# honglu2875/hironaka

Measured on AMD Instinct MI355X. Metric: env-steps/sec at dim=3, max_pts=20, batch=65536; 1/2/4/8 GPUs, higher is better.
Workload: dtype f32

## Files before the change

### hironaka_amd/csrc/hk_duo_kernel.h

```cpp
#pragma once

#include "hk_fast_kernel.h"

namespace hk {

constexpr int kDuoGames = kWave / 2;

__device__ __forceinline__ int duo_other_i(int v) { return qperm_i<0xB1>(v); }
__device__ __forceinline__ float duo_other(float v) { return __int_as_float(duo_other_i(__float_as_int(v))); }

template <int M, int D>
struct DuoGeom {
  using G = FastGeom<M, D>;
  static constexpr int CH = (G::C + 1) / 2;
  static constexpr int QH = (kDuoGames * G::Q + kWave - 1) / kWave;
  static constexpr bool kLean = CH * D <= 30;
};

template <int M, int D>
struct DuoSlabRegs {
  typename VecOf<FastGeom<M, D>::W>::type v[DuoGeom<M, D>::QH];
};

template <int M, int D, bool CONTIG>
__device__ __forceinline__ void duo_slab_issue_impl(DuoSlabRegs<M, D>& r, const float* base, int64_t in_stride,
                                                    int ngames, int lane) {
  using G = FastGeom<M, D>;
  using V = typename VecOf<G::W>::type;
  const int total = ngames * G::Q;
#pragma unroll
  for (int it = 0; it < DuoGeom<M, D>::QH; ++it) {
    int q = lane + it * kWave;
    q = q < total ? q : total - 1;
    r.v[it] = *reinterpret_cast<const V*>(base + slab_chunk_global<M, D, CONTIG>(q, in_stride));
  }
}

template <int M, int D>
__device__ __forceinline__ void duo_slab_issue(DuoSlabRegs<M, D>& r, const float* in, int64_t in_stride, int64_t g0,
                                               int ngames, int lane) {
  const float* base = in + g0 * in_stride;
  if (in_stride == FastGeom<M, D>::N) duo_slab_issue_impl<M, D, true>(r, base, in_stride, ngames, lane);
  else duo_slab_issue_impl<M, D, false>(r, base, in_stride, ngames, lane);
}

template <int M, int D>
__device__ __forceinline__ void duo_slab_commit(DuoSlabRegs<M, D>& r, float* lds, int ngames, int lane) {
  using G = FastGeom<M, D>;
  using V = typename VecOf<G::W>::type;
  const int total = ngames * G::Q;
#pragma unroll
  for (int it = 0; it < DuoGeom<M, D>::QH; ++it) asm volatile("" : "+v"(r.v[it]));
#pragma unroll
  for (int it = 0; it < DuoGeom<M, D>::QH; ++it) {
    const int q = lane + it * kWave;
    if (q < total) *reinterpret_cast<V*>(lds + slab_chunk_lds<M, D>(q)) = r.v[it];
  }
}

constexpr int kStorePlain = 0, kStoreNT = 1, kStoreWT = 2;

template <int M, int D, bool CONTIG, int kBatch, int ST = kStorePlain>
__device__ __forceinline__ void duo_store_slab_impl(const float* lds, float* base, int64_t out_stride, int ngames,
                                                    int lane) {
  using G = FastGeom<M, D>;
  using V = typename VecOf<G::W>::type;
  constexpr int QH = DuoGeom<M, D>::QH;
  constexpr bool kWT = ST == kStoreWT && CONTIG && G::W == 4;
  const int total = ngames * G::Q;
#pragma unroll
  for (int i0 = 0; i0 < QH; i0 += kBatch) {
    V v[kBatch];
#pragma unroll
    for (int u = 0; u < kBatch; ++u) {
      int q = lane + (i0 + u) * kWave;
      q = q < kDuoGames * G::Q ? q : kDuoGames * G::Q - 1;
      v[u] = *reinterpret_cast<const V*>(lds + slab_chunk_lds<M, D>(q));
    }
#pragma unroll
    for (int u = 0; u < kBatch; ++u) asm volatile("" : "+v"(v[u]));
    if constexpr (kWT) {
      typedef unsigned int vu4 __attribute__((ext_vector_type(4)));
      const uint64_t b = (uint64_t)base;
      const uint32_t blo = __builtin_amdgcn_readfirstlane((uint32_t)b), bhi = __builtin_amdgcn_readfirstlane((uint32_t)(b >> 32));
      const int bytes = __builtin_amdgcn_readfirstlane(total * G::W * (int)sizeof(float));
      const auto rsrc = __builtin_amdgcn_make_buffer_rsrc((void*)(((uint64_t)bhi << 32) | blo), 0, bytes, 0x00020000);
#pragma unroll
      for (int u = 0; u < kBatch; ++u) {
        const int q = lane + (i0 + u) * kWave;
        if (i0 + u < QH && q < total)
          __builtin_amdgcn_raw_buffer_store_b128(__builtin_bit_cast(vu4, v[u]), rsrc, q * G::W * (int)sizeof(float), 0,
                                                 16);
      }
    } else {
#pragma unroll
      for (int u = 0; u < kBatch; ++u) {
        const int q = lane + (i0 + u) * kWave;
        if (i0 + u < QH && q < total) {
          V* dst = reinterpret_cast<V*>(base + slab_chunk_global<M, D, CONTIG>(q, out_stride));
          if constexpr (ST != kStorePlain) __builtin_nontemporal_store(v[u], dst);
          else *dst = v[u];
        }
      }
    }
  }
}

template <int M, int D, int kBatch = DuoGeom<M, D>::QH, int ST = kStorePlain>
__device__ inline void duo_store_slab(const float* lds, float* out, int64_t out_stride, int64_t g0, int ngames,
                                      int lane) {
  float* base = out + g0 * out_stride;
  if (out_stride == FastGeom<M, D>::N) duo_store_slab_impl<M, D, true, kBatch, ST>(lds, base, out_stride, ngames, lane);
  else duo_store_slab_impl<M, D, false, kBatch, ST>(lds, base, out_stride, ngames, lane);
}

struct DuoLadder {
  static constexpr int next_bucket(int nb) { return nb < 6 ? nb + 1 : nb + 2; }
};

template <int M, int CH, int D, int SB = CH>
__device__ __forceinline__ void duo_gather_slots(float (&q)[CH * D], const float* mine, uint32_t mask, int smax, int h) {
  mask = h ? (mask & (mask - 1)) : mask;
  unrolled_while<0, SB>([&](auto sc) {
    constexpr int s = decltype(sc)::value;
    if (s >= smax) return false;
    const bool has = mask != 0;
    const float* row = mine + (has ? mask_first(mask) : 0) * D;
    mask &= mask - 1;
    mask &= mask - 1;
#pragma unroll
    for (int k = 0; k < D; ++k) {
      const float v = row[k];
      q[s * D + k] = has ? v : INFINITY;
    }
    return true;
  });
}

template <int CH, int D, int NB, int SB = NB>
__device__ __forceinline__ void duo_gather_level(float (&q)[CH * D], const float* mine, const float* hole, uint32_t mask,
                                                 int h) {
  mask = h ? (mask & (mask - 1)) : mask;
  const float* row[NB];
#pragma unroll
  for (int s = 0; s < NB; ++s) {
    row[s] = mask != 0 ? mine + mask_first(mask) * D : hole;
    mask &= mask - 1;
    mask &= mask - 1;
  }
#pragma unroll
  for (int s = 0; s < NB; ++s)
#pragma unroll
    for (int k = 0; k < D; ++k) q[s * D + k] = row[s][k];
#pragma unroll
  for (int e = NB * D; e < SB * D; ++e) q[e] = INFINITY;
}

template <int M, int CH, int D, bool LEVELS, int SB = CH>
__device__ __forceinline__ void duo_gather(float (&q)[CH * D], const float* mine, const float* hole, uint32_t mask,
                                           int smax, int h) {
  if constexpr (LEVELS) {
    StagesFor<DuoLadder, SB>::run(smax, [&](auto nb) {
      duo_gather_level<CH, D, decltype(nb)::value, SB>(q, mine, hole, mask, h);
      return 0;
    });
  } else {
    duo_gather_slots<M, CH, D, SB>(q, mine, mask, smax, h);
  }
}

template <int CH, int D, int NB>
__device__ __forceinline__ uint32_t duo_scatter_level(const float (&q)[CH * D], float* mine, uint32_t mask, int h) {
  mask = h ? (mask & (mask - 1)) : mask;
  uint32_t alive = 0;
#pragma unroll
  for (int s = 0; s < NB; ++s) {
    if (mask != 0 && q[s * D] < INFINITY) {
      const int slot = mask_first(mask);
      alive |= 1u << slot;
      float* row = mine + slot * D;
#pragma unroll
      for (int k = 0; k < D; ++k) row[k] = q[s * D + k];
    }
    mask &= mask - 1;
    mask &= mask - 1;
  }
  return alive;
}

template <int M, int CH, int D, int SB = CH>
__device__ __forceinline__ uint32_t duo_scatter(const float (&q)[CH * D], float* mine, uint32_t mask, int smax, int h) {
  mask = h ? (mask & (mask - 1)) : mask;
  uint32_t alive = 0;
  unrolled_while<0, SB>([&](auto sc) {
    constexpr int s = decltype(sc)::value;
    if (s >= smax) return false;
    if (mask != 0 && q[s * D] < INFINITY) {
      const int slot = mask_first(mask);
      alive |= 1u << slot;
      float* row = mine + slot * D;
#pragma unroll
      for (int k = 0; k < D; ++k) row[k] = q[s * D + k];
    }
    mask &= mask - 1;
    mask &= mask - 1;
    return true;
  });
  return lanes_or<2>(alive);
}

template <int D>
__device__ __forceinline__ void duo_pad_rows(float* mine, uint32_t dead, float pad, int h) {
  dead = h ? (dead & (dead - 1)) : dead;
  while (dead != 0) {
    float* row = mine + mask_first(dead) * D;
#pragma unroll
    for (int k = 0; k < D; ++k) row[k] = pad;
    dead &= dead - 1;
    dead &= dead - 1;
  }
}

template <int M, int D>
__device__ __forceinline__ void duo_scan_half(const float* mine, float fill, int h, uint32_t& live, bool& ok) {
  static_assert(M <= 32, "the game's mask is one word");
  constexpr int C = (M + 1) / 2;
  const int i0 = h * C;
  const float* base = mine + i0 * D;
  uint32_t mask = 0;
  ok = true;
  const uint32_t fill_bits = __float_as_uint(fill);
#pragma unroll
  for (int r = 0; r < C; ++r) {
    const bool valid = (M % 2 == 0) || r + 1 < C || h == 0;
    uint32_t hi = __float_as_uint(base[r * D]), lo = hi;
#pragma unroll
    for (int k = 1; k < D; ++k) {
      const uint32_t u = __float_as_uint(base[r * D + k]);
      hi = u > hi ? u : hi;
      lo = u < lo ? u : lo;
    }
    const bool ge = hi < 0x7F800000u;
    const bool fl = (lo == fill_bits) && (hi == fill_bits);
    ok &= (ge | fl | !valid);
    mask |= (ge && valid) ? (1u << r) : 0u;
  }
  mask <<= i0;
  live = lanes_or<2>(mask);
}

template <int CH, int D, int NB>
__device__ __forceinline__ void d_newton(float (&q)[CH * D], int h) {
  float acc[NB], oth[NB];
#pragma unroll
  for (int i = 0; i + 1 < NB; ++i) {
#pragma unroll
    for (int j = i + 1; j < NB; ++j) {
      float t, u;
      diff_extrema<D>(&q[i * D], &q[j * D], t, u);
      const float vi = (t > 0.0f) ? -u : 1.0f;
      acc[j] = (i == 0) ? t : hk_fmin(acc[j], t);
      acc[i] = (i == 0 && j == 1) ? vi : hk_fmin(acc[i], vi);
    }
    __builtin_amdgcn_sched_barrier(0);
  }
  const bool late = h != 0;
#pragma unroll
  for (int b = 0; b < NB; ++b) {
    float o[D];
#pragma unroll
    for (int k = 0; k < D; ++k) o[k] = duo_other(q[b * D + k]);
    {
      float t, u;
      diff_extrema<D>(&q[b * D], o, t, u);
      const float va = (t > 0.0f || late) ? -u : 1.0f;
      acc[b] = (NB == 1) ? va : hk_fmin(acc[b], va);
      oth[b] = (u < 0.0f || !late) ? t : 1.0f;
    }
#pragma unroll
    for (int a = 0; a < b; ++a) {
      float t, u;
      diff_extrema<D>(&q[a * D], o, t, u);
      oth[b] = hk_fmin(oth[b], t);
      acc[a] = hk_fmin(acc[a], (t > 0.0f) ? -u : 1.0f);
    }
    __builtin_amdgcn_sched_barrier(0);
  }
#pragma unroll
  for (int r = 0; r < NB; ++r) {
    const bool r0 = acc[r] <= 0.0f, r1 = duo_other(oth[r]) <= 0.0f;
    const bool removed = r0 || r1;
#pragma unroll
    for (int k = 0; k < D; ++k) q[r * D + k] = removed ? INFINITY : q[r * D + k];
  }
}

template <int CH, int D, int NB, bool BIN = false>
__device__ __forceinline__ int d_stages(float (&q)[CH * D], const float (&c)[D], int axis, int np, int h,
                                        unsigned flags, unsigned stages, uint32_t cmask = 0) {
  if (stages & HK_STAGE_SHIFT) {
    if constexpr (BIN) b_shift_mask<CH, D, NB>(q, cmask, axis, np, flags);
    else b_shift<CH, D, NB>(q, c, axis, np, flags);
  }
  if (stages & HK_STAGE_REPOSITION) reposition<2, CH, D, NB, BIN>(q, flags);
  if (stages & HK_STAGE_NEWTON) d_newton<CH, D, NB>(q, h);
  if (stages & HK_STAGE_RESCALE) rescale<2, CH, D, NB>(q, flags);
  return live_rows<2, CH, D, NB>(q);
}

template <int CH, int D, int NB, bool BIN = false>
struct DuoStagesFor {
  static constexpr int kNext = DuoLadder::next_bucket(NB);
  static __device__ __forceinline__ int run(float (&q)[CH * D], int smax, const float (&c)[D], int axis, int np,
                                            int h, unsigned flags, unsigned stages, uint32_t cmask = 0) {
    if constexpr (NB >= CH) {
      return d_stages<CH, D, CH, BIN>(q, c, axis, np, h, flags, stages, cmask);
    } else {
      if (smax <= NB) return d_stages<CH, D, NB, BIN>(q, c, axis, np, h, flags, stages, cmask);
      return DuoStagesFor<CH, D, kNext, BIN>::run(q, smax, c, axis, np, h, flags, stages, cmask);
    }
  }
};

template <int CH, int D>
__device__ __forceinline__ void duo_ranks_first(const float (&q)[CH * D], int smax, int (&rank)[CH]) {
#pragma unroll
  for (int s = 0; s < CH; ++s) rank[s] = 0;
  unrolled_while<0, CH>([&](auto bc) {
    constexpr int b = decltype(bc)::value;
    if (b >= smax) return false;
    float o[D];
#pragma unroll
    for (int k = 0; k < D; ++k) o[k] = duo_other(q[b * D + k]);
    const bool live_o = o[0] < INFINITY, live_b = q[b * D] < INFINITY;
    unrolled_while<0, CH>([&](auto ac) {
      constexpr int a = decltype(ac)::value;
      if (a >= smax) return false;
      rank[a] += (live_o && key_gt<D, kKeyFirst>(o, &q[a * D])) ? 1 : 0;
      if (a != b) rank[a] += (live_b && key_gt<D, kKeyFirst>(&q[b * D], &q[a * D])) ? 1 : 0;
      return true;
    });
    return true;
  });
}

template <int CH, int D>
__device__ __forceinline__ void duo_scatter_ranked(const float (&q)[CH * D], float* mine, const int (&rank)[CH], int smax) {
  unrolled_while<0, CH>([&](auto sc) {
    constexpr int s = decltype(sc)::value;
    if (s >= smax) return false;
    if (q[s * D] < INFINITY) {
      float* row = mine + rank[s] * D;
#pragma unroll
      for (int k = 0; k < D; ++k) row[k] = q[s * D + k];
    }
    return true;
  });
}

struct DuoPolicyCache {
  U4 r;
  uint32_t pair = 0xFFFFFFFFu;
};

__device__ inline void duo_policy_words(uint64_t gg, uint32_t step, uint64_t seed, DuoPolicyCache& cache, int h,
                                        uint32_t& host_word, uint32_t& agent_word) {
  const uint32_t block = step >> 2, pair = block >> 1;
  if (cache.pair != pair) {
    cache.r = philox4x32((uint32_t)gg, (uint32_t)(gg >> 32), (pair << 1) | (uint32_t)h, kStreamPolicy, seed);
    cache.pair = pair;
  }
  const uint32_t mine = u4_word(cache.r, step & 3u);
  const bool own = (int)(block & 1u) == h;
  uint32_t theirs = (uint32_t)duo_other_i((int)mine);
  asm volatile("" : "+v"(theirs));
  const uint32_t w = own ? mine : theirs;
  host_word = w & 0xFFFF0000u;
  agent_word = w << 16;
}

constexpr int kDuoZeilDpp = 6;

template <int CH, int D, int NB>
__device__ __forceinline__ int duo_zeillinger(const float (&q)[CH * D], int h, float* mine, int smax) {
  constexpr bool KEEP = NB <= kDuoZeilDpp;
  ZeilBest<D> best;
#pragma unroll
  for (int k = 0; k < D; ++k) best.bd[k] = 0.0f;
  if constexpr (KEEP) {
    float p[NB * D];
#pragma unroll
    for (int e = 0; e < NB * D; ++e) p[e] = duo_other(q[e]);
#pragma unroll
    for (int a = 0; a < NB; ++a) {
#pragma unroll
      for (int b = a + 1; b < NB; ++b)
        zeil_pair_cmp<D, true, false>(best, &q[a * D], &q[b * D], true, (128 * a + 2 * b) + 65 * h);
#pragma unroll
      for (int b = a; b < NB; ++b)
        zeil_pair_cmp<D, true>(best, &q[a * D], &p[b * D], (b > a) | (h == 0), (128 * a + 2 * b + 1) + 63 * h);
      if constexpr (NB > 3) __builtin_amdgcn_sched_barrier(0);
    }
  } else {
    __syncthreads();
#pragma unroll
    for (int s = 0; s < NB; ++s)
#pragma unroll
      for (int k = 0; k < D; ++k) mine[(2 * s + h) * D + k] = q[s * D + k];
    __syncthreads();
    const int n = 2 * smax;
    ZeilBest<D> second;
#pragma nounroll
    for (int i = h; i + 1 < n; i += 2) {
      float pi[D];
#pragma unroll
      for (int k = 0; k < D; ++k) pi[k] = mine[i * D + k];
#pragma nounroll
      for (int j = i + 1; j < n; j += 2) {
        float pj[D], pk[D];
        const int j2 = (j + 1 < n) ? j + 1 : j;
#pragma unroll
        for (int k = 0; k < D; ++k) {
          pj[k] = mine[j * D + k];
          pk[k] = mine[j2 * D + k];
        }
        zeil_pair2<D>(best, second, pi, pj, 64 * i + j, pi, pk, 64 * i + j + 1);
      }
    }
    zeil_merge<D, false>(best, second);
  }
  {
    ZeilBest<D> o;
    o.hi = (uint32_t)duo_other_i((int)best.hi);
    o.lo = (uint32_t)duo_other_i((int)best.lo);
    if constexpr (KEEP) {
#pragma unroll
      for (int k = 0; k < D; ++k) o.bd[k] = duo_other(best.bd[k]);
    }
    zeil_merge<D, KEEP>(best, o);
  }
  const bool have = best.have();
  if constexpr (!KEEP) {
    const int i = have ? (int)((best.lo & 0xFFFFu) >> 6) : 0, j = have ? (int)(best.lo & 63u) : 0;
#pragma unroll
    for (int k = 0; k < D; ++k) best.bd[k] = mine[i * D + k] - mine[j * D + k];
    __syncthreads();
  }
  int lo = 0, hi = 0;
  float vlo = best.bd[0], vhi = best.bd[0];
#pragma unroll
  for (int k = 1; k < D; ++k) {
    if (best.bd[k] < vlo) { vlo = best.bd[k]; lo = k; }
    if (best.bd[k] > vhi) { vhi = best.bd[k]; hi = k; }
  }
  if (!have || lo == hi) return 0;
  return encode_mask((1u << lo) | (1u << hi));
}

constexpr int kDuoPreBlocks = 6;

template <int D>
__device__ __forceinline__ void duo_policy_fill(uint8_t* act, uint64_t gg, uint32_t wb0, int nb, uint64_t seed,
                                                int host_policy, int agent_policy, int gi, int h) {
  static_assert(D <= 5 && D <= kPolicyShortDim, "an action travels as a byte; four steps per Philox block");
  auto put = [&](const U4& r, int b) {
    int cls, axis;
    uint32_t mask;
#pragma unroll
    for (int k = 0; k < 4; ++k) {
      const uint32_t w = u4_word(r, k);
      policy_from_words<D>(w & 0xFFFF0000u, w << 16, host_policy, agent_policy, cls, axis, mask, 0);
      act[(4 * b + k) * kDuoGames + gi] = (uint8_t)(mask | ((uint32_t)axis << 5));
    }
  };
#pragma nounroll
  for (int i = 0; i < kDuoPreBlocks; i += 4) {
    if (i >= nb) break;
    const int b0 = i + h, b1 = b0 + 2;
    if (i + 2 < nb) {
      const U4 r0 = philox4x32((uint32_t)gg, (uint32_t)(gg >> 32), wb0 + (uint32_t)b0, kStreamPolicy, seed);
      const U4 r1 = philox4x32((uint32_t)gg, (uint32_t)(gg >> 32), wb0 + (uint32_t)b1, kStreamPolicy, seed);
      put(r0, b0);
      if (b1 < kDuoPreBlocks) put(r1, b1);
    } else {
      const U4 r0 = philox4x32((uint32_t)gg, (uint32_t)(gg >> 32), wb0 + (uint32_t)b0, kStreamPolicy, seed);
      if (b0 < kDuoPreBlocks) put(r0, b0);
    }
  }
}

template <int M, int D, int MODE, int HOT = kHotNone, bool ACTS = false, bool ZEIL = false>
__global__ __launch_bounds__(kWave, 2) void duo_kernel(const float* in0, int64_t in_stride0, int batch0,
                                                       const Params prm) {
  static_assert(!ACTS || MODE == kModeRollout, "the small records ride on the plain rollout");
  static_assert(!ZEIL || (MODE == kModeRollout && HOT == kHotNone && !ACTS), "Zeillinger's host: plain rollouts");
  constexpr bool kRec = MODE == kModeRolloutRec;
  constexpr bool kRoll = MODE == kModeRollout || kRec;
  constexpr bool kPartialPublish = MODE == kModeRollout && !ZEIL && DuoGeom<M, D>::kLean;
  constexpr bool kLevelDeal = MODE == kModeRollout && DuoGeom<M, D>::kLean;
  using G = FastGeom<M, D>;
  constexpr int CH = DuoGeom<M, D>::CH;
  static_assert(M <= 32, "the live mask of a game travels as 32 bits");
  __shared__ __align__(16) float lds[kDuoGames * G::S];
  __shared__ float cbuf[kDuoGames * D];
  __shared__ float hole_row[D];
  __shared__ __align__(16) uint8_t pol[(MODE == kModeRollout) ? (4 * kDuoPreBlocks + 1) * kDuoGames : 16];
  const int lane = threadIdx.x;
  const int h = lane & 1, gi = lane >> 1;
  const int64_t g0 = (int64_t)blockIdx.x * kDuoGames;
  const int64_t left = (int64_t)batch0 - g0;
  const int ngames = (int)(left < kDuoGames ? left : kDuoGames);
  const bool active = gi < ngames;
  const bool leader = active && h == 0;
  const int64_t g = g0 + gi;
#ifdef HK_DUO_PROBE
  __shared__ int32_t probe_buf[24];
  if (lane < 24) probe_buf[lane] = 0;
  const long long probe_t0 = wall_clock64();
  long long probe_t1 = 0, probe_t2 = 0;
  int probe_steps = 0, probe_smax = 0;
#endif
  const bool has_ids = kRoll && prm.game_ids != nullptr;
  uint32_t raw_id = 0;
  if (has_ids && active) raw_id = (uint32_t)prm.game_ids[g];
  __builtin_amdgcn_sched_barrier(0);
  DuoSlabRegs<M, D> slab;
  duo_slab_issue<M, D>(slab, in0, in_stride0, g0, ngames, lane);
  __builtin_amdgcn_sched_barrier(0);
  const uint64_t gg = prm.game_offset + (has_ids ? (uint64_t)raw_id : (uint64_t)g);
  uint32_t pol_b0 = prm.step_offset >> 2;
  const uint32_t pol_last = (prm.steps > 0) ? (prm.step_offset + (uint32_t)prm.steps - 1u) >> 2 : pol_b0;
  if constexpr (MODE == kModeRollout && !ZEIL) {
    const uint32_t nb = pol_last - pol_b0 + 1u;
    duo_policy_fill<D>(pol, gg, pol_b0, (int)(nb < (uint32_t)kDuoPreBlocks ? nb : (uint32_t)kDuoPreBlocks), prm.seed,
                       HOT ? (int)HK_HOST_RANDOM : prm.host_policy,
                       (HOT == kHotJax) ? (int)HK_AGENT_RANDOM
                                        : (HOT == kHotTorch) ? (int)HK_AGENT_RANDOM_LEGAL : prm.agent_policy, gi, h);
  }
#ifdef HK_DUO_PROBE
  if (lane == 0) probe_buf[21] = (int32_t)wall_clock64();
#endif
  float* mine = lds + gi * G::S;
  const float pad = (float)prm.pad;
  const unsigned flags = (HOT == kHotJax) ? (unsigned)HK_SEM_JAX : (HOT == kHotTorch) ? kHotTorchFlags : prm.flags;
  const unsigned stages = HOT ? (unsigned)(HK_STAGE_SHIFT | HK_STAGE_REPOSITION | HK_STAGE_NEWTON) : prm.stages;
  const float fill = ((flags & HK_SEM_MASK) == HK_SEM_JAX) ? -1.0f : pad;
  const int nsteps = kRoll ? prm.steps : 1;
  constexpr bool kEndSort = MODE == kModeRollout && HOT == kHotNone;
  const bool end_sort = kEndSort && nsteps > 0 && (stages & HK_STAGE_NEWTON) &&
                        ((flags & HK_SEM_MASK) == HK_SEM_LIST || (flags & HK_FLAG_COMPACT_SORTED));
  bool rescale_pending = false;
  PolicyCache pcache;
  DuoPolicyCache dcache;
  float c[D];
  int axis_in = -1;
#pragma unroll
  for (int k = 0; k < D; ++k) c[k] = 0.0f;
  RawActions<D> raw;
  const bool fetch_actions = !kRoll && (stages & HK_STAGE_SHIFT) && active;
  if (fetch_actions) fast_fetch_actions<D>(prm, g, M, raw);
  duo_slab_commit<M, D>(slab, lds, ngames, lane);
  if (kLevelDeal && lane < D) hole_row[lane] = INFINITY;
  if (fetch_actions) fast_decode_actions<D>(prm, raw, c, axis_in);
  __syncthreads();
#ifdef HK_DUO_PROBE
  if (lane == 0) probe_buf[22] = (int32_t)wall_clock64();
#endif

  uint32_t gmask;
  bool ok;
  duo_scan_half<M, D>(mine, fill, h, gmask, ok);
  if (!active) {
    gmask = 0;
    ok = true;
  }
  int np = mask_pop(gmask);
  int nmax = wave_max(np, M);
  const bool exact = (fill == pad) && __all(ok) && nmax <= G::C;

  if (!exact) {
    float* cs = cbuf + gi * D;
    np = leader ? num_points<float>(mine, M, D) : 2;
    int length = (np < 2) ? 0 : -1;
    if (kRoll && prm.count_ws) {
      const unsigned long long b0 = __ballot(leader && np < 2);
      if (lane == 0) count_add(prm.count_ws + blockIdx.x, (uint32_t)__popcll(b0));
    }
    for (int t = 0; t < nsteps; ++t) {
      int axis = axis_in, cls = 0;
      if (kRec && prm.obs_out) {
        __syncthreads();
        duo_store_slab<M, D, 2>(lds, (float*)prm.obs_out + (int64_t)t * prm.batch * G::N, (int64_t)G::N, g0, ngames, lane);
        __syncthreads();
      }
      if (kRoll) {
        uint32_t mask;
        const int zc = (prm.host_policy == HK_HOST_ZEILLINGER && leader) ? zeillinger_game<float>(mine, prm.m, prm.d) : 0;
        fast_policy<D>(prm, gg, prm.step_offset + (uint32_t)t, pcache, cls, axis, mask, zc);
        if (leader)
          for (int k = 0; k < prm.d; ++k) cs[k] = (float)((mask >> k) & 1u);
      } else if ((stages & HK_STAGE_SHIFT) && leader) {
        load_coords<float>(prm, g, cs);
      }
      const bool prev_done = np < 2;
      if (leader) {
        stages_game<float>(mine, prm.m, prm.d, cs, axis, pad, stages, flags);
        np = num_points<float>(mine, prm.m, prm.d);
      }
      const bool done = np < 2;
      if (done && length < 0) length = t + 1;
      if (kRoll && prm.count_ws) {
        const unsigned long long bd = __ballot(leader && done);
        if (lane == 0) count_add(prm.count_ws + (size_t)(t + 1) * prm.count_stride + blockIdx.x, (uint32_t)__popcll(bd));
      }
      if ((kRec || ACTS) && leader) {
        const int64_t at = (int64_t)t * prm.batch + g;
        if (prm.r_host_class_out) prm.r_host_class_out[at] = cls;
        if (prm.r_axis_out) prm.r_axis_out[at] = axis;
        if (prm.r_done_out) prm.r_done_out[at] = done;
        if (prm.r_reward_out) prm.r_reward_out[at] = prm.reward_sign * (float)(done && !prev_done);
      }
      if (!kRoll && leader) {
        if (prm.done_out) prm.done_out[g] = done;
        if (prm.prev_done_out) prm.prev_done_out[g] = prev_done;
        if (prm.reward_out) prm.reward_out[g] = prm.reward_sign * (float)(done && !prev_done);
        if (prm.num_points_out) prm.num_points_out[g] = np;
      }
    }
    if (kRoll && leader && prm.game_length_out) prm.game_length_out[g] = length;
    __syncthreads();
    duo_store_slab<M, D>(lds, (float*)prm.out, prm.out_stride, g0, ngames, lane);
    return;
  }

  if (kPartialPublish && h == 0) reinterpret_cast<uint32_t*>(cbuf)[gi] = gmask;
  int smax = (nmax + 1) >> 1;
#ifdef HK_DUO_PROBE
  probe_t1 = wall_clock64();
  probe_smax = smax;
#endif
  float q[CH * D];
  if constexpr (!kLevelDeal) {
#pragma unroll
    for (int e = 0; e < CH * D; ++e) q[e] = INFINITY;
  }
  duo_gather<M, CH, D, kLevelDeal>(q, mine, hole_row, gmask, smax, h);
#ifdef HK_DUO_PROBE
  {
    float sink = 0.0f;
#pragma unroll
    for (int e = 0; e < CH * D; ++e) sink += (q[e] < INFINITY) ? q[e] : 0.0f;
    asm volatile("" : "+v"(sink));
    if (lane == 0) probe_buf[23] = (int32_t)wall_clock64();
  }
#endif
  if (!active) np = 2;
  int length = (np < 2) ? 0 : -1;
  if (kRoll && prm.count_ws) {
    const unsigned long long b0 = __ballot(leader && np < 2);
    if (lane == 0) count_add(prm.count_ws + blockIdx.x, (uint32_t)__popcll(b0));
  }
  uint32_t* count_slot = (kRoll && prm.count_ws) ? prm.count_ws + blockIdx.x : nullptr;
  uint32_t count_stride = prm.count_stride;
  uint32_t step0 = prm.step_offset;
  uint64_t seed = prm.seed;
  int host_policy = HOT ? (int)HK_HOST_RANDOM : prm.host_policy;
  int agent_policy = (HOT == kHotJax) ? (int)HK_AGENT_RANDOM
                                      : (HOT == kHotTorch) ? (int)HK_AGENT_RANDOM_LEGAL : prm.agent_policy;
  if (HOT)
    asm volatile("" : "+s"(count_slot), "+s"(count_stride), "+s"(step0), "+s"(seed));
  else
    asm volatile("" : "+s"(count_slot), "+s"(count_stride), "+s"(step0), "+s"(seed), "+s"(host_policy),
                 "+s"(agent_policy));
  static_assert(kDuoGames == 32 && kWave == 64, "flush_records: two steps of the wave's games per instruction");
  int32_t* rec_cls = ACTS ? prm.r_host_class_out : nullptr;
  int32_t* rec_axis = ACTS ? prm.r_axis_out : nullptr;
  uint8_t* rec_done = ACTS ? prm.r_done_out : nullptr;
  float* rec_reward = ACTS ? prm.r_reward_out : nullptr;
  int64_t rec_batch = prm.batch;
  float rec_sign = prm.reward_sign;
  if constexpr (ACTS)
    asm volatile("" : "+s"(rec_cls), "+s"(rec_axis), "+s"(rec_done), "+s"(rec_reward), "+s"(rec_batch), "+s"(rec_sign));
  constexpr bool want_small = ACTS;
  int t_rec = 0;
  auto flush_records = [&](int t_end) {
    if (t_rec < t_end) {
      const int gsel = lane & (kDuoGames - 1), sub = lane >> 5;
      const int lg = __shfl(length, gsel * 2);
      const bool gok = gsel < ngames;
      const int64_t off = (int64_t)sub * rec_batch + gsel;
      const uint8_t* w = pol + (int)(step0 + (uint32_t)t_rec - (pol_b0 << 2)) * kDuoGames + lane;
      for (int ta = t_rec; ta < t_end; ta += 2, w += 2 * kDuoGames) {
        const int tt = ta + sub;
        if (gok && tt < t_end) {
          const uint32_t a = *w;
          const int64_t row = (int64_t)ta * rec_batch + g0;
          if (rec_cls) (rec_cls + row)[off] = encode_mask(a & 31u);
          if (rec_axis) (rec_axis + row)[off] = (int32_t)(a >> 5);
          if (rec_done) (rec_done + row)[off] = lg >= 0 && tt + 1 >= lg;
          if (rec_reward) (rec_reward + row)[off] = rec_sign * (float)(lg >= 1 && tt + 1 == lg);
        }
      }
    }
    t_rec = t_end;
  };
  if constexpr (MODE == kModeRollout) {
    static_assert(CH <= 6 || CH % 2 == 0, "bucket ladder: 1..6, then even numbers");
    int t = 0;
    bool stop = false;
    while (t < nsteps && !stop) {
    if (!ZEIL && (uint32_t)((step0 + (uint32_t)t) >> 2) - pol_b0 >= (uint32_t)kDuoPreBlocks) {
      if constexpr (want_small) flush_records(__builtin_amdgcn_readfirstlane(t));
      __syncthreads();
      pol_b0 = (step0 + (uint32_t)t) >> 2;
      const uint32_t nb = pol_last - pol_b0 + 1u;
      duo_policy_fill<D>(pol, gg, pol_b0, (int)(nb < (uint32_t)kDuoPreBlocks ? nb : (uint32_t)kDuoPreBlocks), seed,
                         host_policy, agent_policy, gi, h);
      __syncthreads();
    }
    const uint32_t wend_abs = (pol_b0 + (uint32_t)kDuoPreBlocks) << 2;
    const int tw = (!ZEIL && wend_abs - step0 < (uint32_t)nsteps) ? (int)(wend_abs - step0) : nsteps;
    uint32_t a_next = ZEIL ? 0u : pol[(int)(step0 + (uint32_t)t - (pol_b0 << 2)) * kDuoGames + gi];
    Levels<DuoLadder, CH>::run([&](auto nbc, auto loc) {
      constexpr int NB = decltype(nbc)::value, LO = decltype(loc)::value;
#ifndef HK_NO_SETPRIO
      if ((smax > LO || LO == 0) && t < tw && !stop) {
        if (t >= 10) __builtin_amdgcn_s_setprio(3);
        else if constexpr (NB >= 6) __builtin_amdgcn_s_setprio(3);
        else if constexpr (NB >= 4) __builtin_amdgcn_s_setprio(2);
        else if constexpr (NB >= 2) __builtin_amdgcn_s_setprio(1);
        else __builtin_amdgcn_s_setprio(0);
      }
#endif
      while (t < tw && (smax > LO || LO == 0) && !stop) {
#ifndef HK_NO_SETPRIO
        if constexpr (NB == 1) {
          if (t == 10) __builtin_amdgcn_s_setprio(3);
        }
#endif
        uint32_t mask;
        int axis;
        if constexpr (ZEIL) {
          static_assert(NB <= kDuoZeilDpp || 2 * NB <= M, "the rolled pair loop parks ranks 0 .. 2 NB - 1 in the game's M rows");
          const int zc = __any(active && np >= 2) ? duo_zeillinger<CH, D, NB>(q, h, mine, smax) : 0;
          uint32_t ra, rb;
          int cls;
          duo_policy_words(gg, step0 + (uint32_t)t, seed, dcache, h, ra, rb);
          policy_from_words<D>(ra, rb, host_policy, agent_policy, cls, axis, mask, zc);
        } else {
          const uint32_t a = a_next;
          a_next = pol[(int)(step0 + (uint32_t)t + 1u - (pol_b0 << 2)) * kDuoGames + gi];
          mask = a & 31u;
          axis = (int)(a >> 5);
        }
        const unsigned st = (end_sort && t + 1 == nsteps) ? (stages & ~(unsigned)HK_STAGE_RESCALE) : stages;
        rescale_pending = end_sort && t + 1 == nsteps && (stages & HK_STAGE_RESCALE);
        np = d_stages<CH, D, NB, true>(q, c, axis, np, h, flags, st, mask);
#ifdef HK_DUO_PROBE
        if (lane == 0 && t == 0) probe_buf[20] = (int32_t)wall_clock64();
#endif
        if (!active) np = 2;
        const bool done = np < 2;
        if (done && length < 0) length = t + 1;
        if constexpr (NB == 1) {
          if (t + 1 < nsteps && !__any(active && !done)) {
            bool still = true;
#pragma unroll
            for (int k = 0; k < D; ++k) still &= (q[k] == 0.0f);
            still |= !(q[0] < INFINITY);
            if (!__any(active && !still)) stop = true;
          }
        } else {
          if (t + 1 < nsteps && !__any(active && ((np + 1) >> 1) >= smax)) {
            __syncthreads();
            if constexpr (kLevelDeal) {
              gmask = lanes_or<2>(duo_scatter_level<CH, D, NB>(q, mine, gmask, h));
              __syncthreads();
              nmax = wave_max(active ? np : 0, 2 * smax - 2);
              smax = (nmax + 1) >> 1;
              duo_gather_level<CH, D, NB>(q, mine, hole_row, gmask, h);
            } else {
              gmask = duo_scatter<M, CH, D, NB>(q, mine, gmask, smax, h);
              __syncthreads();
              const int sprev = smax;
              nmax = wave_max(active ? np : 0, 2 * smax - 2);
              smax = (nmax + 1) >> 1;
              duo_gather_slots<M, CH, D, NB>(q, mine, gmask, sprev, h);
            }
          }
        }
#ifdef HK_DUO_PROBE
        if (lane == 0 && t < 24) probe_buf[t] = (int32_t)((((uint32_t)wall_clock64()) << 4) | (uint32_t)(smax & 15));
#endif
        ++t;
      }
    });
    }
#ifdef HK_DUO_PROBE
    probe_steps = t;
    probe_t2 = wall_clock64();
#endif
    if (count_slot) add_length_counts(count_slot, count_stride, 1, nsteps, leader, length, lane);
    if constexpr (want_small) {
      for (;;) {
        const uint32_t wend = ((pol_b0 + (uint32_t)kDuoPreBlocks) << 2) - step0;
        const int te = __builtin_amdgcn_readfirstlane((wend < (uint32_t)nsteps) ? (int)wend : nsteps);
        flush_records(te);
        if (te >= nsteps) break;
        __syncthreads();
        pol_b0 = (step0 + (uint32_t)te) >> 2;
        const uint32_t nb = pol_last - pol_b0 + 1u;
        duo_policy_fill<D>(pol, gg, pol_b0, (int)(nb < (uint32_t)kDuoPreBlocks ? nb : (uint32_t)kDuoPreBlocks), seed,
                           host_policy, agent_policy, gi, h);
        __syncthreads();
      }
    }
  }
  const bool want_obs = kRec && prm.obs_out != nullptr;
  const bool want_records = kRec && (prm.r_host_class_out || prm.r_axis_out || prm.r_done_out || prm.r_reward_out);
  for (int t = 0; MODE != kModeRollout && t < nsteps; ++t) {
    int axis = axis_in, cls = 0;
    if (want_obs) {
      __syncthreads();
      if (h == 0) fill_image<M, D>(mine, pad);
      __syncthreads();
      duo_scatter<M, CH, D>(q, mine, gmask, smax, h);
      __syncthreads();
      duo_store_slab<M, D, 2>(lds, (float*)prm.obs_out + (int64_t)t * prm.batch * G::N, (int64_t)G::N, g0, ngames, lane);
    }
    uint32_t mask = 0;
    if (kRoll) {
      uint32_t ra, rb;
      duo_policy_words(gg, step0 + (uint32_t)t, seed, dcache, h, ra, rb);
      policy_from_words<D>(ra, rb, host_policy, agent_policy, cls, axis, mask, 0);
    }
    const bool prev_done = np < 2;
    const unsigned st = (end_sort && t + 1 == nsteps) ? (stages & ~(unsigned)HK_STAGE_RESCALE) : stages;
    rescale_pending = end_sort && t + 1 == nsteps && (stages & HK_STAGE_RESCALE);
    np = DuoStagesFor<CH, D, 1, kRoll>::run(q, smax, c, axis, np, h, flags, st, mask);
    if (!active) np = 2;
    const bool done = np < 2;
    if (done && length < 0) length = t + 1;
    if (!kRoll && leader) {
      if (prm.done_out) prm.done_out[g] = done;
      if (prm.prev_done_out) prm.prev_done_out[g] = prev_done;
      if (prm.reward_out) prm.reward_out[g] = prm.reward_sign * (float)(done && !prev_done);
      if (prm.num_points_out) prm.num_points_out[g] = np;
    }
    if (want_records && leader) {
      const int64_t at = (int64_t)t * prm.batch + g;
      if (prm.r_host_class_out) prm.r_host_class_out[at] = cls;
      if (prm.r_axis_out) prm.r_axis_out[at] = axis;
      if (prm.r_done_out) prm.r_done_out[at] = done;
      if (prm.r_reward_out) prm.r_reward_out[at] = prm.reward_sign * (float)(done && !prev_done);
    }
    const unsigned long long bd = __ballot(leader && done);
    if (count_slot && lane == 0) count_add(count_slot + (size_t)(t + 1) * count_stride, (uint32_t)__popcll(bd));
    if (MODE == kModeRollout && smax == 1 && bd == __ballot(leader) && t + 1 < nsteps) {
      bool still = true;
#pragma unroll
      for (int k = 0; k < D; ++k) still &= (q[k] == 0.0f);
      still |= !(q[0] < INFINITY);
      if (!__any(active && !still)) {
        if (count_slot && lane == 0)
          for (int tt = t + 1; tt < nsteps; ++tt) count_add(count_slot + (size_t)(tt + 1) * count_stride, (uint32_t)__popcll(bd));
        break;
      }
    }
    if (t + 1 < nsteps && !__any(active && ((np + 1) >> 1) >= smax)) {
      __syncthreads();
      gmask = duo_scatter<M, CH, D>(q, mine, gmask, smax, h);
      __syncthreads();
      const int sprev = smax;
      nmax = wave_max(active ? np : 0, 2 * smax - 2);
      smax = (nmax + 1) >> 1;
      duo_gather_slots<M, CH, D>(q, mine, gmask, sprev, h);
    }
  }
  if (kRoll && leader && prm.game_length_out) prm.game_length_out[g] = length;

  __syncthreads();
  if (kPartialPublish && !end_sort) {
    const uint32_t alive = duo_scatter<M, CH, D>(q, mine, gmask, smax, h);
    duo_pad_rows<D>(mine, reinterpret_cast<const uint32_t*>(cbuf)[gi] & ~alive, pad, h);
  } else {
    if (h == 0) fill_image<M, D>(mine, pad);
    __syncthreads();
    if (kEndSort && end_sort) {
      int rank[CH];
      duo_ranks_first<CH, D>(q, smax, rank);
      if (rescale_pending) rescale<2, CH, D, CH>(q, flags);
      duo_scatter_ranked<CH, D>(q, mine, rank, smax);
    } else {
      duo_scatter<M, CH, D>(q, mine, gmask, smax, h);
    }
  }
  __syncthreads();
  constexpr int kFinalStore = MODE != kModeRollout ? kStorePlain : DuoGeom<M, D>::kLean ? kStoreWT : kStoreNT;
  duo_store_slab<M, D, DuoGeom<M, D>::QH, kFinalStore>(lds, (float*)prm.out, prm.out_stride, g0, ngames, lane);
#ifdef HK_DUO_PROBE
  if (kRoll && lane == 0 && prm.game_length_out && ngames >= 8) {
    int32_t* w = prm.game_length_out + g0;
    w[0] = (int32_t)probe_t0;
    w[1] = (int32_t)probe_t1;
    w[2] = (int32_t)probe_t2;
    w[3] = (int32_t)wall_clock64();
    w[4] = probe_steps;
    w[5] = probe_smax;
    w[6] = (int32_t)blockIdx.x;
    w[7] = (int32_t)__builtin_amdgcn_s_getreg((4 << 0) | (0 << 6) | (31 << 11));
    if (ngames >= 32)
      for (int i = 0; i < 24; ++i) w[8 + i] = probe_buf[i];
  }
#endif
}

inline int device_simds() {
  static int cached[16] = {0};
  int dev = 0;
  if (hipGetDevice(&dev) != hipSuccess || dev < 0 || dev >= 16) dev = 0;
  if (!cached[dev]) {
    int cus = 0;
    if (hipDeviceGetAttribute(&cus, hipDeviceAttributeMultiprocessorCount, dev) != hipSuccess || cus <= 0) cus = 256;
    (void)hipGetLastError();
    cached[dev] = 4 * cus;
  }
  return cached[dev];
}

inline bool duo_supported(const Params& prm, int dtype) {
  if ((prm.mode != kModeRollout && prm.mode != kModeStep) || prm.m > 32) return false;
  if (prm.mode == kModeStep && (prm.class_out || (prm.stages & kStageFeatureSorts))) return false;
  if (prm.mode == kModeRollout && prm.host_policy == HK_HOST_ZEILLINGER && any_records(prm)) return false;
  if (sorted_output(prm) && (prm.mode != kModeRollout || any_records(prm))) return false;
  return fast_supported(prm, dtype);
}

template <int M, int D>
int launch_duo_t(Params prm, hipStream_t stream) {
  const unsigned grid = (unsigned)(((int64_t)prm.batch + kDuoGames - 1) / kDuoGames);
  prm.games_per_block = kDuoGames;
  launch_prepare();
  const bool records = prm.obs_out != nullptr;
  const bool acts = small_records_only(prm);
  const int hot = (prm.mode == kModeRollout && !records) ? fast_hot_config(prm) : kHotNone;
  if (prm.mode == kModeRollout && records)
    hipLaunchKernelGGL((duo_kernel<M, D, kModeRolloutRec>), dim3(grid), dim3(kWave), 0, stream, (const float*)prm.in,
                       prm.in_stride, prm.batch, prm);
  else if (prm.mode == kModeRollout && prm.host_policy == HK_HOST_ZEILLINGER)
    hipLaunchKernelGGL((duo_kernel<M, D, kModeRollout, kHotNone, false, true>), dim3(grid), dim3(kWave), 0, stream,
                       (const float*)prm.in, prm.in_stride, prm.batch, prm);
  else if (prm.mode == kModeRollout && acts && hot == kHotJax)
    hipLaunchKernelGGL((duo_kernel<M, D, kModeRollout, kHotJax, true>), dim3(grid), dim3(kWave), 0, stream,
                       (const float*)prm.in, prm.in_stride, prm.batch, prm);
  else if (prm.mode == kModeRollout && acts)
    hipLaunchKernelGGL((duo_kernel<M, D, kModeRollout, kHotNone, true>), dim3(grid), dim3(kWave), 0, stream,
                       (const float*)prm.in, prm.in_stride, prm.batch, prm);
  else if (prm.mode == kModeStep && prm.flags == HK_SEM_JAX &&
           prm.stages == (HK_STAGE_SHIFT | HK_STAGE_REPOSITION | HK_STAGE_NEWTON))
    hipLaunchKernelGGL((duo_kernel<M, D, kModeStep, kHotJax>), dim3(grid), dim3(kWave), 0, stream,
                       (const float*)prm.in, prm.in_stride, prm.batch, prm);
  else if (prm.mode == kModeStep)
    hipLaunchKernelGGL((duo_kernel<M, D, kModeStep>), dim3(grid), dim3(kWave), 0, stream, (const float*)prm.in,
                       prm.in_stride, prm.batch, prm);
  else if (hot == kHotJax)
    hipLaunchKernelGGL((duo_kernel<M, D, kModeRollout, kHotJax>), dim3(grid), dim3(kWave), 0, stream,
                       (const float*)prm.in, prm.in_stride, prm.batch, prm);
  else if (hot == kHotTorch)
    hipLaunchKernelGGL((duo_kernel<M, D, kModeRollout, kHotTorch>), dim3(grid), dim3(kWave), 0, stream,
                       (const float*)prm.in, prm.in_stride, prm.batch, prm);
  else
    hipLaunchKernelGGL((duo_kernel<M, D, kModeRollout>), dim3(grid), dim3(kWave), 0, stream, (const float*)prm.in,
                       prm.in_stride, prm.batch, prm);
  return launch_status();
}

#ifndef HK_SPEC_TU
#define HK_X(M_, D_) extern template int launch_duo_t<M_, D_>(Params, hipStream_t);
HK_FAST_SPECS(HK_X)
#undef HK_X

inline int launch_duo(const Params& prm, hipStream_t stream) {
#define HK_X(M_, D_) if (prm.m == M_ && prm.d == D_) return launch_duo_t<M_, D_>(prm, stream);
  HK_FAST_SPECS(HK_X)
#undef HK_X
  return HK_ERR_UNSUPPORTED;
}
#endif

}
```

Before: 58.56 billion.

## Use wave ballots and bitmask shift for the single-row duo rollout tail

Adds a bitmask-based shift (d_shift_words) used in the NB==1 bucket, replacing per-element selects with AND/OR word masks. It also replaces __any reductions with ballots against precomputed active/leader masks, and tracks episode length through a counter instead of per-step branching. The inner loop is split into a play lambda so the setprio switch at step 10 happens once rather than being checked every step. This trades more intricate control flow and liveness bookkeeping (np derived from pair-liveness ballots) for fewer per-step scalar/vector reductions, at some risk of semantic drift in length and done tracking.

```diff
diff --git a/hironaka_amd/csrc/hk_duo_kernel.h b/hironaka_amd/csrc/hk_duo_kernel.h
--- a/hironaka_amd/csrc/hk_duo_kernel.h
+++ b/hironaka_amd/csrc/hk_duo_kernel.h
@@ -8,6 +8,8 @@
 
 __device__ __forceinline__ int duo_other_i(int v) { return qperm_i<0xB1>(v); }
 __device__ __forceinline__ float duo_other(float v) { return __int_as_float(duo_other_i(__float_as_int(v))); }
+
+__device__ __forceinline__ uint64_t duo_ballot(bool p) { return __builtin_amdgcn_ballot_w64(p); }
 
 template <int M, int D>
 struct DuoGeom {
@@ -295,11 +297,37 @@
   }
 }
 
-template <int CH, int D, int NB, bool BIN = false>
+template <int CH, int D, int NB>
+__device__ __forceinline__ void d_shift_words(float (&q)[CH * D], uint32_t cmask, int axis, int np, unsigned flags) {
+  bool apply = true;
+  if (flags & HK_FLAG_AXIS_NOOP_IF_INVALID) apply = axis >= 0 && ((cmask >> axis) & 1u);
+  if ((flags & HK_FLAG_IGNORE_ENDED) && np < 2) apply = false;
+  const uint32_t onehot = apply ? 1u << (axis & 31) : 0u;
+  uint32_t isax[D], in[D];
+#pragma unroll
+  for (int k = 0; k < D; ++k) {
+    isax[k] = (uint32_t)((int32_t)(onehot << (31 - k)) >> 31);
+    in[k] = (uint32_t)((int32_t)(cmask << (31 - k)) >> 31);
+    asm volatile("" : "+v"(isax[k]), "+v"(in[k]));
+  }
+#pragma unroll
+  for (int r = 0; r < NB; ++r) {
+    float s = __uint_as_float(__float_as_uint(q[r * D]) & in[0]);
+#pragma unroll
+    for (int k = 1; k < D; ++k) s = s + __uint_as_float(__float_as_uint(q[r * D + k]) & in[k]);
+#pragma unroll
+    for (int k = 0; k < D; ++k)
+      q[r * D + k] = __uint_as_float((__float_as_uint(s) & isax[k]) | (__float_as_uint(q[r * D + k]) & ~isax[k]));
+  }
+}
+
+template <int CH, int D, int NB, bool BIN = false, bool WORDS = false>
 __device__ __forceinline__ int d_stages(float (&q)[CH * D], const float (&c)[D], int axis, int np, int h,
                                         unsigned flags, unsigned stages, uint32_t cmask = 0) {
+  static_assert(!WORDS || BIN, "the subset as bits");
   if (stages & HK_STAGE_SHIFT) {
-    if constexpr (BIN) b_shift_mask<CH, D, NB>(q, cmask, axis, np, flags);
+    if constexpr (WORDS) d_shift_words<CH, D, NB>(q, cmask, axis, np, flags);
+    else if constexpr (BIN) b_shift_mask<CH, D, NB>(q, cmask, axis, np, flags);
     else b_shift<CH, D, NB>(q, c, axis, np, flags);
   }
   if (stages & HK_STAGE_REPOSITION) reposition<2, CH, D, NB, BIN>(q, flags);
@@ -706,11 +734,18 @@
   };
   if constexpr (MODE == kModeRollout) {
     static_assert(CH <= 6 || CH % 2 == 0, "bucket ladder: 1..6, then even numbers");
+    uint64_t amask = duo_ballot(active), lmask = duo_ballot(leader);
+    asm volatile("" : "+s"(amask), "+s"(lmask));
+    int open_steps = (np < 2) ? -1 : 0;
+    auto length_at = [&](int tt) { return open_steps == tt ? -1 : open_steps + 1; };
     int t = 0;
     bool stop = false;
     while (t < nsteps && !stop) {
     if (!ZEIL && (uint32_t)((step0 + (uint32_t)t) >> 2) - pol_b0 >= (uint32_t)kDuoPreBlocks) {
-      if constexpr (want_small) flush_records(__builtin_amdgcn_readfirstlane(t));
+      if constexpr (want_small) {
+        length = length_at(t);
+        flush_records(__builtin_amdgcn_readfirstlane(t));
+      }
       __syncthreads();
       pol_b0 = (step0 + (uint32_t)t) >> 2;
       const uint32_t nb = pol_last - pol_b0 + 1u;
@@ -723,79 +758,97 @@
     uint32_t a_next = ZEIL ? 0u : pol[(int)(step0 + (uint32_t)t - (pol_b0 << 2)) * kDuoGames + gi];
     Levels<DuoLadder, CH>::run([&](auto nbc, auto loc) {
       constexpr int NB = decltype(nbc)::value, LO = decltype(loc)::value;
+      if (!((smax > LO || LO == 0) && t < tw && !stop)) return;
 #ifndef HK_NO_SETPRIO
-      if ((smax > LO || LO == 0) && t < tw && !stop) {
-        if (t >= 10) __builtin_amdgcn_s_setprio(3);
-        else if constexpr (NB >= 6) __builtin_amdgcn_s_setprio(3);
-        else if constexpr (NB >= 4) __builtin_amdgcn_s_setprio(2);
-        else if constexpr (NB >= 2) __builtin_amdgcn_s_setprio(1);
-        else __builtin_amdgcn_s_setprio(0);
-      }
-#endif
-      while (t < tw && (smax > LO || LO == 0) && !stop) {
-#ifndef HK_NO_SETPRIO
-        if constexpr (NB == 1) {
-          if (t == 10) __builtin_amdgcn_s_setprio(3);
-        }
-#endif
-        uint32_t mask;
-        int axis;
-        if constexpr (ZEIL) {
-          static_assert(NB <= kDuoZeilDpp || 2 * NB <= M, "the rolled pair loop parks ranks 0 .. 2 NB - 1 in the game's M rows");
-          const int zc = __any(active && np >= 2) ? duo_zeillinger<CH, D, NB>(q, h, mine, smax) : 0;
-          uint32_t ra, rb;
-          int cls;
-          duo_policy_words(gg, step0 + (uint32_t)t, seed, dcache, h, ra, rb);
-          policy_from_words<D>(ra, rb, host_policy, agent_policy, cls, axis, mask, zc);
-        } else {
-          const uint32_t a = a_next;
-          a_next = pol[(int)(step0 + (uint32_t)t + 1u - (pol_b0 << 2)) * kDuoGames + gi];
-          mask = a & 31u;
-          axis = (int)(a >> 5);
-        }
-        const unsigned st = (end_sort && t + 1 == nsteps) ? (stages & ~(unsigned)HK_STAGE_RESCALE) : stages;
-        rescale_pending = end_sort && t + 1 == nsteps && (stages & HK_STAGE_RESCALE);
-        np = d_stages<CH, D, NB, true>(q, c, axis, np, h, flags, st, mask);
+      if (t >= 10) __builtin_amdgcn_s_setprio(3);
+      else if constexpr (NB >= 6) __builtin_amdgcn_s_setprio(3);
+      else if constexpr (NB >= 4) __builtin_amdgcn_s_setprio(2);
+      else if constexpr (NB >= 2) __builtin_amdgcn_s_setprio(1);
+      else __builtin_amdgcn_s_setprio(0);
+#endif
+      auto play = [&](int tend) {
+        while (t < tend) {
+          uint32_t mask;
+          int axis;
+          if constexpr (ZEIL) {
+            static_assert(NB <= kDuoZeilDpp || 2 * NB <= M, "the rolled pair loop parks ranks 0 .. 2 NB - 1 in the game's M rows");
+            const int zc = (duo_ballot(np >= 2) & amask) != 0 ? duo_zeillinger<CH, D, NB>(q, h, mine, smax) : 0;
+            uint32_t ra, rb;
+            int cls;
+            duo_policy_words(gg, step0 + (uint32_t)t, seed, dcache, h, ra, rb);
+            policy_from_words<D>(ra, rb, host_policy, agent_policy, cls, axis, mask, zc);
+          } else {
+            const uint32_t a = a_next;
+            a_next = pol[(int)(step0 + (uint32_t)t + 1u - (pol_b0 << 2)) * kDuoGames + gi];
+            mask = a & 31u;
+            axis = (int)(a >> 5);
+          }
+          const unsigned st = (end_sort && t + 1 == nsteps) ? (stages & ~(unsigned)HK_STAGE_RESCALE) : stages;
+          rescale_pending = end_sort && t + 1 == nsteps && (stages & HK_STAGE_RESCALE);
+          const int np_new = d_stages<CH, D, NB, true, (NB == 1)>(q, c, axis, np, h, flags, st, mask);
 #ifdef HK_DUO_PROBE
-        if (lane == 0 && t == 0) probe_buf[20] = (int32_t)wall_clock64();
-#endif
-        if (!active) np = 2;
-        const bool done = np < 2;
-        if (done && length < 0) length = t + 1;
-        if constexpr (NB == 1) {
-          if (t + 1 < nsteps && !__any(active && !done)) {
-            bool still = true;
-#pragma unroll
-            for (int k = 0; k < D; ++k) still &= (q[k] == 0.0f);
-            still |= !(q[0] < INFINITY);
-            if (!__any(active && !still)) stop = true;
-          }
-        } else {
-          if (t + 1 < nsteps && !__any(active && ((np + 1) >> 1) >= smax)) {
-            __syncthreads();
-            if constexpr (kLevelDeal) {
-              gmask = lanes_or<2>(duo_scatter_level<CH, D, NB>(q, mine, gmask, h));
-              __syncthreads();
-              nmax = wave_max(active ? np : 0, 2 * smax - 2);
-              smax = (nmax + 1) >> 1;
-              duo_gather_level<CH, D, NB>(q, mine, hole_row, gmask, h);
-            } else {
-              gmask = duo_scatter<M, CH, D, NB>(q, mine, gmask, smax, h);
-              __syncthreads();
-              const int sprev = smax;
-              nmax = wave_max(active ? np : 0, 2 * smax - 2);
-              smax = (nmax + 1) >> 1;
-              duo_gather_slots<M, CH, D, NB>(q, mine, gmask, sprev, h);
+          if (lane == 0 && t == 0) probe_buf[20] = (int32_t)wall_clock64();
+#endif
+          if constexpr (NB == 1) {
+            const uint64_t live = duo_ballot(q[0] < INFINITY);
+            const uint64_t open = live & (live >> 1) & lmask;
+            open_steps += __builtin_amdgcn_inverse_ballot_w64(open) ? 1 : 0;
+            np = __builtin_amdgcn_inverse_ballot_w64(open | (open << 1)) ? 2 : 0;
+            if (open == 0) {
+              uint32_t any_bits = __float_as_uint(q[0]);
+#pragma unroll
+              for (int k = 1; k < D; ++k) any_bits |= __float_as_uint(q[k]);
+              if ((duo_ballot(any_bits != 0u) & live & amask) == 0) {
+                stop = true;
+                tend = 0;
+              }
+            }
+          } else {
+            np = np_new;
+            open_steps += (leader && np >= 2) ? 1 : 0;
+            if ((duo_ballot(np >= 2 * smax - 1) & amask) == 0) {
+              int left = nsteps - 1 - t;
+              asm volatile("" : "+s"(left));
+              if (left > 0) {
+                __syncthreads();
+                if constexpr (kLevelDeal) {
+                  gmask = lanes_or<2>(duo_scatter_level<CH, D, NB>(q, mine, gmask, h));
+                  __syncthreads();
+                  nmax = wave_max(active ? np : 0, 2 * smax - 2);
+                  smax = (nmax + 1) >> 1;
+                  duo_gather_level<CH, D, NB>(q, mine, hole_row, gmask, h);
+                } else {
+                  gmask = duo_scatter<M, CH, D, NB>(q, mine, gmask, smax, h);
+                  __syncthreads();
+                  const int sprev = smax;
+                  nmax = wave_max(active ? np : 0, 2 * smax - 2);
+                  smax = (nmax + 1) >> 1;
+                  duo_gather_slots<M, CH, D, NB>(q, mine, gmask, sprev, h);
+                }
+                tend = smax <= LO ? 0 : tend;
+              }
             }
           }
+#ifdef HK_DUO_PROBE
+          if (lane == 0 && t < 24) probe_buf[t] = (int32_t)((((uint32_t)wall_clock64()) << 4) | (uint32_t)(smax & 15));
+#endif
+          ++t;
         }
-#ifdef HK_DUO_PROBE
-        if (lane == 0 && t < 24) probe_buf[t] = (int32_t)((((uint32_t)wall_clock64()) << 4) | (uint32_t)(smax & 15));
-#endif
-        ++t;
+      };
+      if constexpr (NB == 1) {
+        play(tw < 10 ? tw : 10);
+        if (t < tw && !stop) {
+#ifndef HK_NO_SETPRIO
+          __builtin_amdgcn_s_setprio(3);
+#endif
+          play(tw);
+        }
+      } else {
+        play(tw);
       }
     });
     }
+    length = length_at(t);
 #ifdef HK_DUO_PROBE
     probe_steps = t;
     probe_t2 = wall_clock64();
```

New measurement: 62.09 billion, median of 6. +6.0%, better.
